# dayne-2stacks/Fingerprint-Matching-Code

Measured on AMD Instinct MI355X. Metric: graph-match pairs/sec @ n=256 kpts, batch=1024, 1 & 8 GPU, higher is better.
Workload: dtype bf16

## Files before the change

fingerprint-matching-code_amd/csrc/gemm.hip:

```cpp
#include "gemm_phase.h"
#include <cstdlib>
#include <cstring>

namespace fpm {
int& gemm_bn256_min();
}
int& gemm_store_sc1_flag();

extern "C" int fpm_gemm(int dtype, const void* A, long lda, long sA, const int* a_rows, const void* B, long ldb,
                        long sB, int M, int N, int K, int batch, int epi, const float* bias, float* Cf, void* Ct,
                        long ldc, long sC, const int* n1, const int* n2, void* stream) {
    using namespace fpm;
    FPM_CHECK_ARG(dtype == 0 || dtype == 1, "gemm: dtype must be 0 (f32) or 1 (bf16)");
    FPM_CHECK_ARG(M >= 0 && N > 0 && K > 0 && batch >= 0, "gemm: bad sizes M=%d N=%d K=%d", M, N, K);
    FPM_CHECK_ARG(K % (dtype ? 8 : 4) == 0, "gemm: K=%d must be a multiple of %d", K, dtype ? 8 : 4);
    FPM_CHECK_ARG(lda % (dtype ? 8 : 4) == 0 && ldb % (dtype ? 8 : 4) == 0, "gemm: lda/ldb must keep rows 16-B aligned");
    FPM_CHECK_ARG((epi != EPI_AFFINITY && epi != EPI_HALF_AFFINITY) || (n1 && n2),
                  "gemm: affinity epilogues need n1/n2");
    FPM_CHECK_ARG(epi >= EPI_STORE && epi <= EPI_HALF_AFFINITY, "gemm: bad epilogue %d", epi);
    if (M == 0 || batch == 0) return 0;
    GemmParams p = {};
    p.A = A; p.lda = lda; p.sA = sA; p.a_rows = a_rows;
    p.B = B; p.ldb = ldb; p.sB = sB; p.sB_seg = 0;
    p.row_scale = nullptr;
// ... 2 lines not shown
    p.epi = epi; p.bias = bias; p.Cf = Cf; p.Ct = Ct; p.ldc = ldc; p.sC = sC; p.n1 = n1; p.n2 = n2;
    hipStream_t st = (hipStream_t)stream;
    const int mt = (M + G2_BM - 1) / G2_BM;
    const bool epi_ok = epi == EPI_STORE || epi == EPI_RELU || (epi == EPI_AFFINITY && Cf && !Ct);
    const bool big = dtype == 1 && M >= G2_BM && K % G2_BK == 0 && N % 8 == 0 && lda % 8 == 0 && ldb % 8 == 0 &&
                     !(Cf && Ct) && (Cf ? ldc % 4 == 0 : ldc % 8 == 0) && epi_ok &&
                     (long)mt * ((N + 127) / 128) * batch >= 128;
    if (big) {
        const int BN = (N % 256 == 0 && (long)mt * (N / 256) * batch >= gemm_bn256_min()) ? 256 : 128;
        p.remap_mtiles = mt;
        dim3 grid(remap_grid_big(N, BN, mt), 1, batch);
        const bool f32 = Cf != nullptr;
        const bool phase = BN == 256 && use_gemm_phase(K);
#define FPM_BIG(BN_, E_, F_)                                                                            \
    do {                                                                                               \
        if (BN_ == 256 && phase) hipLaunchKernelGGL((gemm_phase_kernel<E_, F_>), grid, dim3(G2_THREADS), 0, st, p); \
        else hipLaunchKernelGGL((gemm_big_kernel<BN_, E_, F_>), grid, dim3(G2_THREADS), 0, st, p);      \
    } while (0)
        if (epi == EPI_AFFINITY) {
            if (BN == 256) FPM_BIG(256, EPI_AFFINITY, true); else FPM_BIG(128, EPI_AFFINITY, true);
        } else if (BN == 256) {
            if (epi == EPI_RELU) { if (f32) FPM_BIG(256, EPI_RELU, true); else FPM_BIG(256, EPI_RELU, false); }
            else if (f32) FPM_BIG(256, EPI_STORE, true);
            else {
                const int S = phase ? gemm_walk_strip(p) : 0;
                p.store_sc1 = gemm_store_sc1_flag();
                if (S != 0) gemm_walk_launch(p, S, batch, st);
                else FPM_BIG(256, EPI_STORE, false);
            }
        } else {
            if (epi == EPI_RELU) { if (f32) FPM_BIG(128, EPI_RELU, true); else FPM_BIG(128, EPI_RELU, false); }
// ... 10 lines not shown
}

namespace fpm {
int& gemm_phase_flag() {
    static int on = [] {
        const char* e = getenv("FPM_GEMM_PHASE");
        return e ? atoi(e) : 1;
    }();
    return on;
}

int& gemm_walk_flag() {
    static int v = [] {
        const char* e = getenv("FPM_GEMM_WALK");
        return e ? atoi(e) : GW_AUTO;
    }();
    return v;
}

int gemm_cu_count() {
    static int cus = [] {
        int dev = 0, n = 0;
        if (hipGetDevice(&dev) != hipSuccess ||
            hipDeviceGetAttribute(&n, hipDeviceAttributeMultiprocessorCount, dev) != hipSuccess || n <= 0)
            n = 256;
        return n;
    }();
    return cus;
}

// ... 127 lines not shown
int& gnn_store_sc1_flag();
int& combine_store_sc1_flag();
int& gemm_store_sc1_flag();
int& combine_lds_kb_flag();
int& gnn_mlp_off_flag();
int& outer_sum_vec_flag();
int& gnn_sweeps_flag();
int& scatter_f32_rows_flag();
int& scatter_batch_flag();
int& afau_head_split_flag();

extern "C" int fpm_set_tuning(const char* key, int value) {
    int* f = nullptr;
    if (key && !strcmp(key, "gemm_phase")) f = &fpm::gemm_phase_flag();
    else if (key && !strcmp(key, "gemm_walk")) f = &fpm::gemm_walk_flag();
    else if (key && !strcmp(key, "gemm_bn256_min")) f = &fpm::gemm_bn256_min();
    else if (key && !strcmp(key, "plan_graph")) f = &plan_graph_flag();
    else if (key && !strcmp(key, "combine_npb")) f = &combine_npb_flag();
    else if (key && !strcmp(key, "sinkhorn_bwd_reg")) f = &sinkhorn_bwd_reg_flag();
    else if (key && !strcmp(key, "sinkhorn_fast")) f = &sinkhorn_fast_flag();
    else if (key && !strcmp(key, "sinkhorn_lform")) f = &sinkhorn_lform_flag();
    else if (key && !strcmp(key, "topk_fast")) f = &soft_topk_fast_flag();
    else if (key && !strcmp(key, "afau_attn_v")) f = &afau_attn_v_flag();
    else if (key && !strcmp(key, "gnn_store_sc1")) f = &gnn_store_sc1_flag();
    else if (key && !strcmp(key, "combine_store_sc1")) f = &combine_store_sc1_flag();
    else if (key && !strcmp(key, "gemm_store_sc1")) f = &gemm_store_sc1_flag();
    else if (key && !strcmp(key, "combine_lds_kb")) f = &combine_lds_kb_flag();
    else if (key && !strcmp(key, "gnn_mlp_off")) f = &gnn_mlp_off_flag();
    else if (key && !strcmp(key, "outer_sum_vec")) f = &outer_sum_vec_flag();
    else if (key && !strcmp(key, "gnn_sweeps")) f = &gnn_sweeps_flag();
// ... 175 lines not shown
```

fingerprint-matching-code_amd/csrc/gemm_phase.h:

```cpp
#pragma once
#include <type_traits>
#include "gemm_big.h"

namespace fpm {

constexpr int GP_HALF = 128 * 128;
constexpr int GP_SMEM = g2_max(8 * GP_HALF, G2_BM * (2 * 256 + 16));
constexpr int GP_MIN_KTILES = 2;

#define FPM_VMCNT(N) asm volatile("s_waitcnt vmcnt(" #N ")" ::: "memory")

#ifdef GP_PROBE
__device__ unsigned long long* gp_probe_buf;
#define GP_STAMP(k)                                                                                   \
    do {                                                                                              \
        const unsigned long long t_ = __builtin_amdgcn_s_memtime();                                   \
        if (threadIdx.x == 0 && gp_probe_buf)                                                         \
            gp_probe_buf[((long)blockIdx.z * gridDim.x + blockIdx.x) * 8 + (k)] = t_;                   \
    } while (0)
#else
#define GP_STAMP(k)
#endif

#ifndef GP_STAGGER
#define GP_STAGGER 1
#endif
#ifndef GP_PRIO
#define GP_PRIO 1
#endif
template <int EPI, bool F32OUT, bool DIRECT = false>
__global__ __launch_bounds__(G2_THREADS, 1) void gemm_phase_kernel(GemmParams p) {
    constexpr int BN = 256;
    __shared__ __attribute__((aligned(16))) unsigned char smem[GP_SMEM];
    const int tid = threadIdx.x, lane = tid & 63, wave = tid >> 6;
    const int wr = wave >> 2, wc = wave & 3;
    const int batch = blockIdx.z;

    const int nt = (p.N + BN - 1) / BN;
    const int q = remap_tile(nt, p.remap_mtiles, p.remap_cm > 0 ? p.remap_cm : 4);
    const int mtile = q / nt, ntile = q - mtile * nt;
    if (mtile >= p.remap_mtiles) return;
    int group = 0, row0, row_end;
    if (p.tile_info) {
        group = p.tile_info[2 * mtile];
        if (group < 0) return;
        row0 = p.tile_info[2 * mtile + 1];
        row_end = p.group_off[group + 1];
    } else {
        row0 = mtile * G2_BM;
        row_end = p.M;
// ... 7 lines not shown
    for (int i = 0; i < 2; ++i) {
        const int r = (wave * 2 + i) * 8 + (lane >> 3);
        const int kc = (lane & 7) ^ ((r >> 1) & 7);
#pragma unroll
        for (int h = 0; h < 2; ++h) {
            int gr = row0 + h * 128 + r;
            gr = gr < row_end ? gr : row0;
            const long arow = p.a_rows ? (long)p.a_rows[gr] : (long)gr;
            src[h][i] = A + arow * p.lda + kc * 8;
            const int n = n0 + h * 128 + r < p.N ? n0 + h * 128 + r : p.N - 1;
            src[2 + h][i] = Bg + (long)n * p.ldb + kc * 8;
        }
    }
    auto issue = [&](int j, int slot) {
        const int t = j >> 2;
        unsigned char* dst = smem + ((t & 1) * 4 + slot) * GP_HALF + wave * 2048;
        const int k0 = t * G2_BK;
        __builtin_amdgcn_global_load_lds((gbl_ptr_t)(src[slot][0] + k0), (lds_ptr_t)dst, 16, 0, 0);
        __builtin_amdgcn_global_load_lds((gbl_ptr_t)(src[slot][1] + k0), (lds_ptr_t)(dst + 1024), 16, 0, 0);
    };

    const int xr = (lane >> 1) & 7;
    const int a_off = (wr * 64 + (lane & 15)) * 128;
    const int b_off = (wc * 32 + (lane & 15)) * 128;
    const int s0 = ((lane >> 4) ^ xr) * 16, s1 = ((4 + (lane >> 4)) ^ xr) * 16;

    f32x4_t acc[2][2][4][2];
#pragma unroll
    for (int h = 0; h < 2; ++h)
#pragma unroll
        for (int g = 0; g < 2; ++g)
#pragma unroll
            for (int i = 0; i < 4; ++i)
#pragma unroll
                for (int j = 0; j < 2; ++j) acc[h][g][i][j] = f32x4_t{0.f, 0.f, 0.f, 0.f};
    bf16x8_t a[2][4], b0[2][2], b1[2][2];

    auto read_a = [&](int t, int h) {
        const unsigned char* base = smem + ((t & 1) * 4 + h) * GP_HALF + a_off;
#pragma unroll
        for (int f = 0; f < 4; ++f) {
            a[0][f] = *(const bf16x8_t*)(base + f * 2048 + s0);
            a[1][f] = *(const bf16x8_t*)(base + f * 2048 + s1);
        }
    };
    auto read_b = [&](int t, int g, bf16x8_t (&bb)[2][2]) {
        const unsigned char* base = smem + ((t & 1) * 4 + 2 + g) * GP_HALF + b_off;
#pragma unroll
        for (int f = 0; f < 2; ++f) {
            bb[0][f] = *(const bf16x8_t*)(base + f * 2048 + s0);
            bb[1][f] = *(const bf16x8_t*)(base + f * 2048 + s1);
        }
    };
    auto mfma = [&](f32x4_t (&c)[4][2], bf16x8_t (&bb)[2][2]) {
        __builtin_amdgcn_s_barrier();
        asm volatile("s_waitcnt lgkmcnt(0)" ::: "memory");
        if (GP_PRIO) __builtin_amdgcn_s_setprio(1);
#pragma unroll
        for (int kk = 0; kk < 2; ++kk)
#pragma unroll
            for (int fm = 0; fm < 4; ++fm)
#pragma unroll
                for (int fn = 0; fn < 2; ++fn) {
                    if constexpr (DIRECT)
                        c[fm][fn] = __builtin_amdgcn_mfma_f32_16x16x32_bf16(bb[kk][fn], a[kk][fm], c[fm][fn], 0, 0, 0);
                    else
                        c[fm][fn] = __builtin_amdgcn_mfma_f32_16x16x32_bf16(a[kk][fm], bb[kk][fn], c[fm][fn], 0, 0, 0);
                }
        if (GP_PRIO) __builtin_amdgcn_s_setprio(0);
        __builtin_amdgcn_s_barrier();
    };
    constexpr int SLOT[4] = {0, 2, 3, 1};
    auto ktile = [&](int t, auto VM0, auto VM1, auto VM2, auto VM3, bool iss0, bool iss1, bool iss2, bool iss3) {
        const int phi = 4 * t;
        if constexpr (decltype(VM0)::value == 6) FPM_VMCNT(6);
        else if constexpr (decltype(VM0)::value == 4) FPM_VMCNT(4);
        else if constexpr (decltype(VM0)::value == 2) FPM_VMCNT(2);
        else if constexpr (decltype(VM0)::value == 0) FPM_VMCNT(0);
        if (iss0) issue(phi + 6, SLOT[(0 + 6) & 3]);
        read_a(t, 0);
        read_b(t, 0, b0);
        mfma(acc[0][0], b0);
        if constexpr (decltype(VM1)::value == 6) FPM_VMCNT(6);
        else if constexpr (decltype(VM1)::value == 4) FPM_VMCNT(4);
        else if constexpr (decltype(VM1)::value == 2) FPM_VMCNT(2);
        else if constexpr (decltype(VM1)::value == 0) FPM_VMCNT(0);
        if (iss1) issue(phi + 7, SLOT[(1 + 6) & 3]);
        read_b(t, 1, b1);
        mfma(acc[0][1], b1);
        if constexpr (decltype(VM2)::value == 6) FPM_VMCNT(6);
        else if constexpr (decltype(VM2)::value == 4) FPM_VMCNT(4);
        else if constexpr (decltype(VM2)::value == 2) FPM_VMCNT(2);
        else if constexpr (decltype(VM2)::value == 0) FPM_VMCNT(0);
        if (iss2) issue(phi + 8, SLOT[(2 + 6) & 3]);
        read_a(t, 1);
        mfma(acc[1][1], b1);
        if constexpr (decltype(VM3)::value == 6) FPM_VMCNT(6);
        else if constexpr (decltype(VM3)::value == 4) FPM_VMCNT(4);
        else if constexpr (decltype(VM3)::value == 2) FPM_VMCNT(2);
        else if constexpr (decltype(VM3)::value == 0) FPM_VMCNT(0);
        if (iss3) issue(phi + 9, SLOT[(3 + 6) & 3]);
        mfma(acc[1][0], b0);
    };
    using V6 = std::integral_constant<int, 6>;
    using V4 = std::integral_constant<int, 4>;
    using V2 = std::integral_constant<int, 2>;
    using V0 = std::integral_constant<int, 0>;
    using VN = std::integral_constant<int, -1>;

    GP_STAMP(0);
    const int ktiles = p.K / G2_BK;
#pragma unroll
    for (int j = 0; j < 6; ++j) issue(j, SLOT[j & 3]);
    FPM_VMCNT(8);
    __builtin_amdgcn_s_barrier();
    GP_STAMP(1);
    if (GP_STAGGER && wr == 1) __builtin_amdgcn_s_barrier();

    int t = 0;
    for (; t < ktiles - 2; ++t) ktile(t, V6{}, V6{}, V6{}, V6{}, true, true, true, true);
    ktile(t, V6{}, V6{}, V6{}, V4{}, true, true, false, false);
    ktile(t + 1, V2{}, V0{}, VN{}, VN{}, false, false, false, false);
    if (GP_STAGGER && wr == 0) __builtin_amdgcn_s_barrier();
    __syncthreads();
    GP_STAMP(2);

    int n1b = 0, n2b = 0;
    if (EPI == EPI_AFFINITY) { n1b = p.n1[batch]; n2b = p.n2[batch]; }
    if constexpr (DIRECT) {
        static_assert(!F32OUT && EPI == EPI_STORE, "DIRECT: bf16 output, plain store");
        bf16_t* Ct = (bf16_t*)p.Ct + (long)batch * p.sC;
        const int cl = wc * 32 + 4 * (lane >> 4);
#pragma unroll
        for (int h = 0; h < 2; ++h)
#pragma unroll
            for (int fm = 0; fm < 4; ++fm) {
                const int r = row0 + h * 128 + wr * 64 + fm * 16 + (lane & 15);
// ... 125 lines not shown

constexpr int GW_SMEM = 8 * GP_HALF;
constexpr int GW_MAX_S = 2;

__host__ __device__ inline int gemm_walk_rule(int tiles, int wgs, int cus) {
    const long r1 = ((long)tiles * wgs + cus - 1) / cus, r2 = ((long)((tiles + 1) / 2) * wgs + cus - 1) / cus;
    return 2 * r2 * 7 <= r1 * 8 ? 2 : 1;
}

#ifdef GP_PROBE
#define GW_STAMP(k) do { if (ti == 0) GP_STAMP(k); } while (0)
#else
#define GW_STAMP(k)
#endif

template <bool SC1>
__global__ __launch_bounds__(G2_THREADS, 1) void gemm_walk_kernel(GemmParams p) {
    constexpr int BN = 256;
    __shared__ __attribute__((aligned(16))) unsigned char smem[GW_SMEM];
    const int tid = threadIdx.x, lane = tid & 63, wave = tid >> 6;
    const int wr = wave >> 2, wc = wave & 3;
    const int batch = blockIdx.z;

    const int nt = p.N / BN;
    int mtiles = p.remap_mtiles;
    if (p.tile_count) mtiles = *p.tile_count < mtiles ? *p.tile_count : mtiles;
    const int S = p.walk > 0 ? p.walk : gemm_walk_rule(mtiles, nt * (int)gridDim.z, p.walk_cus);
    const int strips = (mtiles + S - 1) / S;
    const int i = blockIdx.x >> 3;
    const int strip = (i / nt) * 8 + (blockIdx.x & 7), ntile = i % nt;
    if (strip >= strips) return;
    int t_row0[GW_MAX_S], t_rend[GW_MAX_S], t_grp[GW_MAX_S];
    unsigned ok = 0;
#pragma unroll
    for (int j = 0; j < GW_MAX_S; ++j) {
        const int mt = strip * S + j;
// ... 23 lines not shown
    auto pick = [&](const int (&t)[GW_MAX_S], int j) __attribute__((always_inline)) {
        return j == 0 ? t[0] : t[1];
    };
    int m = next_valid(0);

    const int n0 = ntile * BN;
    const bf16_t* A = (const bf16_t*)p.A + (long)batch * p.sA;
    const unsigned char* Bb = (const unsigned char*)((const bf16_t*)p.B + (long)batch * p.sB);
    bf16_t* Ct = (bf16_t*)p.Ct + (long)batch * p.sC;

    auto tile_at = [&](int j, int& row0, int& row_end, const unsigned char*& bg) __attribute__((always_inline)) {
        row0 = pick(t_row0, j);
        row_end = pick(t_rend, j);
        bg = Bb + (long)pick(t_grp, j) * p.sB_seg * 2;
    };
    auto a_rows_of = [&](int row0, int row_end, int (&ar)[2][2]) __attribute__((always_inline)) {
#pragma unroll
        for (int i = 0; i < 2; ++i)
#pragma unroll
            for (int h = 0; h < 2; ++h) {
                int gr = row0 + h * 128 + (wave * 2 + i) * 8 + (lane >> 3);
                gr = gr < row_end ? gr : row0;
                ar[h][i] = p.a_rows ? p.a_rows[gr] : gr;
            }
    };
    const uint32_t kc16 = (uint32_t)(((lane & 7) ^ (lane >> 4)) * 16);
    uint32_t b_off[2];
#pragma unroll
    for (int i = 0; i < 2; ++i)
        b_off[i] = (uint32_t)((n0 + (wave * 2 + i) * 8 + (lane >> 3)) * (uint32_t)p.ldb * 2) + (kc16 ^ (i * 64));
    const uint32_t lda2 = (uint32_t)p.lda * 2, bhalf = 128 * (uint32_t)p.ldb * 2;
    const unsigned char* Ab = (const unsigned char*)A;

    int row0, row_end, row0n = 0, row_endn = 0;
    const unsigned char *bg, *bgn = nullptr;
    int ar[2][2], arn[2][2];

    auto issue = [&](int slot, int buf, const int (&rows)[2][2], const unsigned char* bgrp, int k0) __attribute__((always_inline)) {
        unsigned char* dst = smem + (buf * 4 + slot) * GP_HALF + wave * 2048;
        if (slot < 2) {
            const unsigned char* ab = Ab + 2 * k0;
#pragma unroll
            for (int i = 0; i < 2; ++i)
                __builtin_amdgcn_global_load_lds(
                    (gbl_ptr_t)(ab + ((uint64_t)(uint32_t)rows[slot][i] * lda2 + (kc16 ^ (i * 64)))),
                    (lds_ptr_t)(dst + i * 1024), 16, 0, 0);
        } else {
            const unsigned char* b = bgrp + 2 * k0 + (slot - 2) * bhalf;
            __builtin_amdgcn_global_load_lds((gbl_ptr_t)(b + b_off[0]), (lds_ptr_t)dst, 16, 0, 0);
            __builtin_amdgcn_global_load_lds((gbl_ptr_t)(b + b_off[1]), (lds_ptr_t)(dst + 1024), 16, 0, 0);
        }
    };

    const int xr = (lane >> 1) & 7;
    const int a_off = (wr * 64 + (lane & 15)) * 128;
    const int b_offl = (wc * 32 + (lane & 15)) * 128;
    const int s0 = ((lane >> 4) ^ xr) * 16, s1 = ((4 + (lane >> 4)) ^ xr) * 16;

    f32x4_t acc[2][2][4][2];
    auto zero_acc = [&]() __attribute__((always_inline)) {
#pragma unroll
        for (int h = 0; h < 2; ++h)
#pragma unroll
            for (int g = 0; g < 2; ++g)
#pragma unroll
                for (int i = 0; i < 4; ++i)
#pragma unroll
                    for (int j = 0; j < 2; ++j) acc[h][g][i][j] = f32x4_t{0.f, 0.f, 0.f, 0.f};
    };
    bf16x8_t a[2][4], b0[2][2], b1[2][2];

    auto read_a = [&](int u, int h) __attribute__((always_inline)) {
        const unsigned char* base = smem + ((u & 1) * 4 + h) * GP_HALF + a_off;
#pragma unroll
        for (int f = 0; f < 4; ++f) {
            a[0][f] = *(const bf16x8_t*)(base + f * 2048 + s0);
            a[1][f] = *(const bf16x8_t*)(base + f * 2048 + s1);
        }
    };
    auto read_b = [&](int u, int g, bf16x8_t (&bb)[2][2]) __attribute__((always_inline)) {
        const unsigned char* base = smem + ((u & 1) * 4 + 2 + g) * GP_HALF + b_offl;
#pragma unroll
        for (int f = 0; f < 2; ++f) {
            bb[0][f] = *(const bf16x8_t*)(base + f * 2048 + s0);
            bb[1][f] = *(const bf16x8_t*)(base + f * 2048 + s1);
        }
    };
    auto mfma = [&](f32x4_t (&c)[4][2], bf16x8_t (&bb)[2][2]) __attribute__((always_inline)) {
        __builtin_amdgcn_s_barrier();
        asm volatile("s_waitcnt lgkmcnt(0)" ::: "memory");
        if (GP_PRIO) __builtin_amdgcn_s_setprio(1);
#pragma unroll
        for (int kk = 0; kk < 2; ++kk)
#pragma unroll
            for (int fm = 0; fm < 4; ++fm)
#pragma unroll
                for (int fn = 0; fn < 2; ++fn)
                    c[fm][fn] = __builtin_amdgcn_mfma_f32_16x16x32_bf16(bb[kk][fn], a[kk][fm], c[fm][fn], 0, 0, 0);
        if (GP_PRIO) __builtin_amdgcn_s_setprio(0);
        __builtin_amdgcn_s_barrier();
    };
    constexpr int NONE = 0, CUR = 1, NEXT = 2;
    auto wait = [&](int v) __attribute__((always_inline)) {
        if (v == 6) FPM_VMCNT(6);
        else if (v == 4) FPM_VMCNT(4);
        else if (v == 2) FPM_VMCNT(2);
        else if (v == 0) FPM_VMCNT(0);
    };
    auto iss = [&](int mode, int slot, int buf, int k0) __attribute__((always_inline)) {
        if (mode == CUR) issue(slot, buf, ar, bg, k0);
        else if (mode == NEXT) issue(slot, buf, arn, bgn, 0);
    };
    auto ktile = [&](int u, int k1, int VM0, int VM1, int VM2, int VM3, int M01, int M23) __attribute__((always_inline)) {
        asm volatile("" : "+s"(k1));
        wait(VM0);
        iss(M01, 3, (u + 1) & 1, k1);
        read_a(u, 0);
        read_b(u, 0, b0);
        mfma(acc[0][0], b0);
        wait(VM1);
        iss(M01, 1, (u + 1) & 1, k1);
        read_b(u, 1, b1);
        mfma(acc[0][1], b1);
        wait(VM2);
        iss(M23, 0, u & 1, k1 + G2_BK);
        read_a(u, 1);
        mfma(acc[1][1], b1);
        wait(VM3);
        iss(M23, 2, u & 1, k1 + G2_BK);
        mfma(acc[1][0], b0);
    };

    auto epilogue = [&](int buf, auto hb) __attribute__((always_inline)) {
        constexpr bool HB = decltype(hb)::value;
        unsigned char* img = smem + buf * (4 * GP_HALF);
        int tid_ = tid;
        asm volatile("" : "+v"(tid_));
        const int lane = tid_ & 63, wr = tid_ >> 8, wc = (tid_ >> 6) & 3;
        int wbase[2];
#pragma unroll
        for (int fn = 0; fn < 2; ++fn)
            wbase[fn] = (wr * 64 + (lane & 15)) * 512 + (((wc * 4 + fn * 2 + (lane >> 5)) ^ (lane & 7)) << 4) +
                        ((lane >> 4) & 1) * 8;
        const int rb_r = tid_ >> 5, rb_c = tid_ & 31;
        const int rbase = rb_r * 512 + ((rb_c ^ (rb_r & 7)) << 4);
// ... 32 lines not shown
                    }
                }
            } else {
#pragma unroll
                for (int it = 0; it < 8; ++it) {
                    const uint4 v = *(const uint4*)(img + rbase + it * 8192);
                    if (rbeg + it * 16 < row_end) *(uint4*)(Ct + (long)(rbeg + it * 16) * p.ldc + n0 + rb_c * 8) = v;
                }
            }
            asm volatile("s_waitcnt lgkmcnt(0)" ::: "memory");
            __builtin_amdgcn_s_barrier();
        }
    };

    const int T = p.K / G2_BK;
    tile_at(m, row0, row_end, bg);
    a_rows_of(row0, row_end, ar);
    int mn = next_valid(m + 1);
    if (mn < m_end) {
        tile_at(mn, row0n, row_endn, bgn);
        a_rows_of(row0n, row_endn, arn);
    }
    issue(0, 0, ar, bg, 0);
    issue(2, 0, ar, bg, 0);
    issue(3, 0, ar, bg, 0);
    issue(1, 0, ar, bg, 0);
    issue(0, 1, ar, bg, G2_BK);
    issue(2, 1, ar, bg, G2_BK);
    zero_acc();
    FPM_VMCNT(8);
    __builtin_amdgcn_s_barrier();

    int u = 0;
#ifdef GP_PROBE
    int ti = 0;
#endif
    for (;;) {
        const bool has_next = mn < m_end;
        GW_STAMP(0);
        if (GP_STAGGER && wr == 1) __builtin_amdgcn_s_barrier();
        int k1 = G2_BK;
        for (int t = 0; t < T - 2; ++t, ++u, k1 += G2_BK) ktile(u, k1, 6, 6, 6, 6, CUR, CUR);
        ktile(u, k1, 6, 6, 6, has_next ? 6 : 4, CUR, has_next ? NEXT : NONE);
        GW_STAMP(1);
        ktile(u + 1, 0, has_next ? 6 : 2, has_next ? 6 : 0, -1, -1, has_next ? NEXT : NONE, NONE);
        ++u;
        if (GP_STAGGER && wr == 0) __builtin_amdgcn_s_barrier();
        GW_STAMP(2);
        if (p.bias) epilogue(u & 1, std::true_type{});
        else epilogue(u & 1, std::false_type{});
        GW_STAMP(3);
        if (!has_next) break;
        m = mn; mn = m_end;
        row0 = row0n; row_end = row_endn; bg = bgn;
#pragma unroll
        for (int h = 0; h < 2; ++h)
#pragma unroll
            for (int i = 0; i < 2; ++i) ar[h][i] = arn[h][i];
        issue(0, u & 1, ar, bg, G2_BK);
        issue(2, u & 1, ar, bg, G2_BK);
        FPM_VMCNT(4);
        zero_acc();
        __builtin_amdgcn_s_barrier();
        GW_STAMP(4);
        ++u;
#ifdef GP_PROBE
        ++ti;
#endif
    }
}

#undef FPM_VMCNT

int& gemm_phase_flag();
inline bool use_gemm_phase(int K) { return gemm_phase_flag() != 0 && K / G2_BK >= GP_MIN_KTILES; }

constexpr int GW_AUTO = 8;
int& gemm_walk_flag();
int gemm_cu_count();
inline int gemm_walk_strip(const GemmParams& p) {
    const int f = gemm_walk_flag();
    if (f <= 1 || !use_gemm_phase(p.K) || p.N % 256 != 0 || !p.Ct || p.Cf || p.epi != EPI_STORE) return 0;
    if ((long)p.N * p.ldb * 2 >= (1L << 31) || (long)G2_BM * p.ldc * 2 >= (1L << 31) || p.lda >= (1L << 31)) return 0;
    return f < GW_AUTO ? 2 : GW_AUTO;
}
inline void gemm_walk_launch(GemmParams p, int S, int batch, hipStream_t st) {
    const long nt = p.N / 256;
    p.walk_cus = gemm_cu_count();
    p.walk = S == 2 || p.remap_mtiles * nt * batch >= 8L * gemm_cu_count() ? 2 : 0;
    const int strips = p.walk ? (p.remap_mtiles + 1) / 2 : p.remap_mtiles;
    const dim3 grid((unsigned)((strips + 7) / 8 * 8 * nt), 1, batch);
    if (p.store_sc1) hipLaunchKernelGGL((gemm_walk_kernel<true>), grid, dim3(G2_THREADS), 0, st, p);
    else hipLaunchKernelGGL((gemm_walk_kernel<false>), grid, dim3(G2_THREADS), 0, st, p);
}

}
```

fingerprint-matching-code_amd/csrc/spline.hip:

```cpp
#include "gemm_phase.h"

#include <vector>

namespace {

struct ProfRec {
    hipEvent_t a, b;
    int slot;
};
bool g_prof_on = false;
std::vector<ProfRec> g_prof;
int* g_prof_rows = nullptr;
constexpr int PROF_MAX = 4096;

constexpr int NCELL = 26;

struct PlanLayout {
    long mask, indeg, dslot, basis_e, grp_e, blk_cnt, cell_off, rowid, arows, tile_info, tile_info2, dst_ptr, csr_e,
        nbr_local, rows4, basis4, total;
    long nblk, max_rows, max_tiles, max_tiles2;
};

__host__ __device__ inline long al(long x) { return (x + 255) & ~255L; }

// ... 1134 lines not shown
        if (dtype == 1) p.tile_info = (const int*)(w + L.tile_info2);
        const int walk = dtype == 1 ? gemm_walk_strip(p) : 0;
        p.tile_count = (const int*)(w + L.cell_off) + NCELL + 2;
        dim3 grid(dtype == 0 ? remap_grid(D, p.remap_mtiles) : remap_grid256(D, p.remap_mtiles), 1, 1);
        ProfRec rec = {nullptr, nullptr, (int)g_prof.size()};
        if (g_prof_on && !g_prof_rows) (void)hipMalloc(&g_prof_rows, PROF_MAX * sizeof(int));
        if (g_prof_on && g_prof_rows && rec.slot < PROF_MAX) {
            (void)hipMemcpyAsync(g_prof_rows + rec.slot, w + L.cell_off + NCELL * sizeof(int), sizeof(int),
                                 hipMemcpyDeviceToDevice, st);
            (void)hipEventCreate(&rec.a);
            (void)hipEventCreate(&rec.b);
            (void)hipEventRecord(rec.a, st);
        }
        if (dtype == 0) hipLaunchKernelGGL((gemm_kernel<float, false>), grid, dim3(GTHREADS), 0, st, p);
        else if (walk != 0) gemm_walk_launch(p, walk, 1, st);
        else if (use_gemm_phase(D)) hipLaunchKernelGGL((gemm_phase_kernel<EPI_STORE, false>), grid, dim3(G2_THREADS), 0, st, p);
        else hipLaunchKernelGGL((gemm_big_kernel<256, EPI_STORE, false>), grid, dim3(G2_THREADS), 0, st, p);
        if (g_prof_on && g_prof_rows && rec.slot < PROF_MAX) {
            (void)hipEventRecord(rec.b, st);
            g_prof.push_back(rec);
        }
    }
    {
        const long graphs = (num_nodes + nmax - 1) / nmax;
        const int npb = combine_npb_flag();
#define FPM_COMB(T_, N_)                                                                                         \
    do {                                                                                                         \
        const dim3 cg((unsigned)(((graphs + 7) / 8) * 8 * ((nmax + N_ - 1) / N_)));                              \
        const size_t lds = (size_t)combine_lds_kb_flag() * 1024;                                                 \
        if (combine_store_sc1_flag() && !(mode >> 1))                                                            \
            hipLaunchKernelGGL((combine_kernel<T_, N_, false, 16>), cg, dim3(64 * N_), lds, st, (const T_*)y_ws, \
// ... 328 lines not shown
    }
    GemmParams p = {};
    p.A = dtype == 0 ? (const void*)dY : (const void*)dY_op; p.lda = D; p.a_rows = nullptr;
    p.B = Wb; p.ldb = D; p.sB_seg = (long)D * D;
    p.M = (int)L.max_rows; p.N = D; p.K = D; p.nseg = 1;
    p.group_off = (const int*)(w + L.cell_off);
    p.epi = EPI_STORE; p.ldc = D; p.Cf = dXrows;
    if (dtype == 0) {
        p.tile_info = (const int*)(w + L.tile_info);
        p.remap_mtiles = (int)L.max_tiles;
        hipLaunchKernelGGL((gemm_kernel<float, false>), dim3(remap_grid(D, p.remap_mtiles)), dim3(GTHREADS), 0, st, p);
    } else {
        p.tile_info = (const int*)(w + L.tile_info2);
        p.remap_mtiles = (int)L.max_tiles2;
        dim3 grid(remap_grid256(D, p.remap_mtiles));
        if (use_gemm_phase(D)) hipLaunchKernelGGL((gemm_phase_kernel<EPI_STORE, true>), grid, dim3(G2_THREADS), 0, st, p);
        else hipLaunchKernelGGL((gemm_big_kernel<256, EPI_STORE, true>), grid, dim3(G2_THREADS), 0, st, p);
    }
    hipLaunchKernelGGL(node_rows_sum_kernel, dim3(nb), dim3(256), 0, st, dXrows, (const int*)(w + L.rowid), num_nodes,
                       accumulate, dX);
    return check_launch("fpm_spline_conv_bwd_data");
}

namespace {

template <typename TO, bool TRANS>
__global__ __launch_bounds__(256) void spline_w_pack_kernel(const float* __restrict__ weight,
                                                            const float* __restrict__ root, int K, int Cin, int Cout,
                                                            TO* __restrict__ out) {
    __shared__ float t[64][65];
    const int k = blockIdx.z;
// ... 40 lines not shown
```

Measured before the change: 32570.

## Balance LDS reads across GEMM phase quarters by prefetching next B tile

Reorders the global-to-LDS stream slots and moves the first B-fragment read of each k-tile into the previous k-tile's last quarter. This spreads LDS reads more evenly across the four MFMA phases. B register buffers alternate between k-tiles through a swap flag, and an odd/even prologue handles the tile count parity. The phase and walk kernels now share a common k-tile helper. A probe-only per-phase clock is added, and the balanced variant is on by default through a new FPM_GEMM_BALANCE flag. The risk is extra register pressure and subtle pipeline hazards from the reordered slot timing.

```diff
diff --git a/fingerprint-matching-code_amd/csrc/gemm.hip b/fingerprint-matching-code_amd/csrc/gemm.hip
--- a/fingerprint-matching-code_amd/csrc/gemm.hip
+++ b/fingerprint-matching-code_amd/csrc/gemm.hip
@@ -40,7 +40,7 @@
         const bool phase = BN == 256 && use_gemm_phase(K);
 #define FPM_BIG(BN_, E_, F_)                                                                            \
     do {                                                                                               \
-        if (BN_ == 256 && phase) hipLaunchKernelGGL((gemm_phase_kernel<E_, F_>), grid, dim3(G2_THREADS), 0, st, p); \
+        if (BN_ == 256 && phase) gemm_phase_launch<E_, F_>(p, grid, st);                                \
         else hipLaunchKernelGGL((gemm_big_kernel<BN_, E_, F_>), grid, dim3(G2_THREADS), 0, st, p);      \
     } while (0)
         if (epi == EPI_AFFINITY) {
@@ -81,6 +81,14 @@
     static int v = [] {
         const char* e = getenv("FPM_GEMM_WALK");
         return e ? atoi(e) : GW_AUTO;
+    }();
+    return v;
+}
+
+int& gemm_balance_flag() {
+    static int v = [] {
+        const char* e = getenv("FPM_GEMM_BALANCE");
+        return e ? atoi(e) : 1;
     }();
     return v;
 }
@@ -238,6 +246,7 @@
     int* f = nullptr;
     if (key && !strcmp(key, "gemm_phase")) f = &fpm::gemm_phase_flag();
     else if (key && !strcmp(key, "gemm_walk")) f = &fpm::gemm_walk_flag();
+    else if (key && !strcmp(key, "gemm_balance")) f = &fpm::gemm_balance_flag();
     else if (key && !strcmp(key, "gemm_bn256_min")) f = &fpm::gemm_bn256_min();
     else if (key && !strcmp(key, "plan_graph")) f = &plan_graph_flag();
     else if (key && !strcmp(key, "combine_npb")) f = &combine_npb_flag();
diff --git a/fingerprint-matching-code_amd/csrc/gemm_phase.h b/fingerprint-matching-code_amd/csrc/gemm_phase.h
--- a/fingerprint-matching-code_amd/csrc/gemm_phase.h
+++ b/fingerprint-matching-code_amd/csrc/gemm_phase.h
@@ -18,8 +18,51 @@
         if (threadIdx.x == 0 && gp_probe_buf)                                                         \
             gp_probe_buf[((long)blockIdx.z * gridDim.x + blockIdx.x) * 8 + (k)] = t_;                   \
     } while (0)
+__device__ unsigned* gp_phase_buf;
+struct GpClock {
+    unsigned last, sum[4][3], n;
+    static __device__ __forceinline__ unsigned now() {
+        unsigned long long t;
+        __builtin_amdgcn_sched_barrier(0);
+        asm volatile("s_memtime %0\n\ts_waitcnt lgkmcnt(0)" : "=s"(t)::"memory");
+        __builtin_amdgcn_sched_barrier(0);
+        return (unsigned)t;
+    }
+    __device__ __forceinline__ void start() {
+        n = 0;
+#pragma unroll
+        for (int q = 0; q < 4; ++q)
+#pragma unroll
+            for (int k = 0; k < 3; ++k) sum[q][k] = 0;
+        last = now();
+    }
+    __device__ __forceinline__ void resume() { last = now(); }
+    __device__ __forceinline__ void mark(int q, int part) {
+        const unsigned t = now();
+        sum[q][part] += t - last;
+        last = t;
+    }
+    __device__ __forceinline__ void ktile_done() { ++n; }
+    __device__ __forceinline__ void store() const {
+        if ((threadIdx.x & 255) == 0 && gp_phase_buf) {
+            unsigned* o = gp_phase_buf + (((long)blockIdx.z * gridDim.x + blockIdx.x) * 2 + (threadIdx.x >> 8)) * 16;
+#pragma unroll
+            for (int q = 0; q < 4; ++q)
+#pragma unroll
+                for (int k = 0; k < 3; ++k) o[q * 3 + k] = sum[q][k];
+            o[12] = n;
+        }
+    }
+};
 #else
 #define GP_STAMP(k)
+struct GpClock {
+    __device__ __forceinline__ void start() {}
+    __device__ __forceinline__ void resume() {}
+    __device__ __forceinline__ void mark(int, int) {}
+    __device__ __forceinline__ void ktile_done() {}
+    __device__ __forceinline__ void store() const {}
+};
 #endif
 
 #ifndef GP_STAGGER
@@ -28,12 +71,100 @@
 #ifndef GP_PRIO
 #define GP_PRIO 1
 #endif
-template <int EPI, bool F32OUT, bool DIRECT = false>
+
+__device__ __forceinline__ void gp_wait(int v) {
+    if (v == 6) FPM_VMCNT(6);
+    else if (v == 4) FPM_VMCNT(4);
+    else if (v == 2) FPM_VMCNT(2);
+    else if (v == 0) FPM_VMCNT(0);
+}
+
+template <bool SWAP>
+struct GpTile {
+    const unsigned char* smem;
+    int a_off, b_off, s0, s1;
+    __device__ __forceinline__ GpTile(const unsigned char* sm, int lane, int wr, int wc) : smem(sm) {
+        const int xr = (lane >> 1) & 7;
+        a_off = (wr * 64 + (lane & 15)) * 128;
+        b_off = (wc * 32 + (lane & 15)) * 128;
+        s0 = ((lane >> 4) ^ xr) * 16;
+        s1 = ((4 + (lane >> 4)) ^ xr) * 16;
+    }
+    __device__ __forceinline__ void read_a(int u, int h, bf16x8_t (&a)[2][4]) const {
+        const unsigned char* base = smem + ((u & 1) * 4 + h) * GP_HALF + a_off;
+#pragma unroll
+        for (int f = 0; f < 4; ++f) {
+            a[0][f] = *(const bf16x8_t*)(base + f * 2048 + s0);
+            a[1][f] = *(const bf16x8_t*)(base + f * 2048 + s1);
+        }
+    }
+    __device__ __forceinline__ void read_b(int u, int g, bf16x8_t (&bb)[2][2]) const {
+        const unsigned char* base = smem + ((u & 1) * 4 + 2 + g) * GP_HALF + b_off;
+#pragma unroll
+        for (int f = 0; f < 2; ++f) {
+            bb[0][f] = *(const bf16x8_t*)(base + f * 2048 + s0);
+            bb[1][f] = *(const bf16x8_t*)(base + f * 2048 + s1);
+        }
+    }
+    __device__ __forceinline__ void mfma(GpClock& clk, int q, f32x4_t (&c)[4][2], const bf16x8_t (&a)[2][4],
+                                         const bf16x8_t (&bb)[2][2]) const {
+        __builtin_amdgcn_s_barrier();
+        asm volatile("s_waitcnt lgkmcnt(0)" ::: "memory");
+        clk.mark(q, 1);
+        if (GP_PRIO) __builtin_amdgcn_s_setprio(1);
+#pragma unroll
+        for (int kk = 0; kk < 2; ++kk)
+#pragma unroll
+            for (int fm = 0; fm < 4; ++fm)
+#pragma unroll
+                for (int fn = 0; fn < 2; ++fn) {
+                    if constexpr (SWAP)
+                        c[fm][fn] = __builtin_amdgcn_mfma_f32_16x16x32_bf16(bb[kk][fn], a[kk][fm], c[fm][fn], 0, 0, 0);
+                    else
+                        c[fm][fn] = __builtin_amdgcn_mfma_f32_16x16x32_bf16(a[kk][fm], bb[kk][fn], c[fm][fn], 0, 0, 0);
+                }
+        if (GP_PRIO) __builtin_amdgcn_s_setprio(0);
+        __builtin_amdgcn_s_barrier();
+        clk.mark(q, 2);
+    }
+};
+
+template <bool BAL>
+__device__ __forceinline__ constexpr int gp_stream_slot(int pos) {
+    return pos == 0 ? (BAL ? 2 : 0) : pos == 1 ? (BAL ? 0 : 2) : pos == 2 ? 3 : 1;
+}
+
+template <bool BAL, bool SWAP, class Stage>
+__device__ __forceinline__ void gp_ktile(const GpTile<SWAP>& T, GpClock& clk, int u, bool pre, Stage&& stage,
+                                         f32x4_t (&acc)[2][2][4][2], bf16x8_t (&a)[2][4], bf16x8_t (&bx)[2][2],
+                                         bf16x8_t (&by)[2][2]) {
+    stage(std::integral_constant<int, 0>{});
+    clk.mark(0, 0);
+    T.read_a(u, 0, a);
+    if constexpr (!BAL) T.read_b(u, 0, bx);
+    T.mfma(clk, 0, acc[0][0], a, bx);
+    stage(std::integral_constant<int, 1>{});
+    clk.mark(1, 0);
+    T.read_b(u, 1, by);
+    T.mfma(clk, 1, acc[0][1], a, by);
+    stage(std::integral_constant<int, 2>{});
+    clk.mark(2, 0);
+    T.read_a(u, 1, a);
+    T.mfma(clk, 2, acc[1][1], a, by);
+    stage(std::integral_constant<int, 3>{});
+    clk.mark(3, 0);
+    if (BAL && pre) T.read_b(u + 1, 0, by);
+    T.mfma(clk, 3, acc[1][0], a, bx);
+    clk.ktile_done();
+}
+
+template <int EPI, bool F32OUT, bool DIRECT = false, bool BAL = true>
 __global__ __launch_bounds__(G2_THREADS, 1) void gemm_phase_kernel(GemmParams p) {
     constexpr int BN = 256;
     __shared__ __attribute__((aligned(16))) unsigned char smem[GP_SMEM];
     const int tid = threadIdx.x, lane = tid & 63, wave = tid >> 6;
     const int wr = wave >> 2, wc = wave & 3;
+    const int wave_s = __builtin_amdgcn_readfirstlane(wave);
     const int batch = blockIdx.z;
 
     const int nt = (p.N + BN - 1) / BN;
@@ -71,17 +202,14 @@
     }
     auto issue = [&](int j, int slot) {
         const int t = j >> 2;
-        unsigned char* dst = smem + ((t & 1) * 4 + slot) * GP_HALF + wave * 2048;
+        unsigned char* dst = smem + ((t & 1) * 4 + slot) * GP_HALF + wave_s * 2048;
         const int k0 = t * G2_BK;
         __builtin_amdgcn_global_load_lds((gbl_ptr_t)(src[slot][0] + k0), (lds_ptr_t)dst, 16, 0, 0);
         __builtin_amdgcn_global_load_lds((gbl_ptr_t)(src[slot][1] + k0), (lds_ptr_t)(dst + 1024), 16, 0, 0);
     };
 
-    const int xr = (lane >> 1) & 7;
-    const int a_off = (wr * 64 + (lane & 15)) * 128;
-    const int b_off = (wc * 32 + (lane & 15)) * 128;
-    const int s0 = ((lane >> 4) ^ xr) * 16, s1 = ((4 + (lane >> 4)) ^ xr) * 16;
-
+    const GpTile<DIRECT> T(smem, lane, wr, wc);
+    GpClock clk;
     f32x4_t acc[2][2][4][2];
 #pragma unroll
     for (int h = 0; h < 2; ++h)
@@ -93,91 +221,44 @@
                 for (int j = 0; j < 2; ++j) acc[h][g][i][j] = f32x4_t{0.f, 0.f, 0.f, 0.f};
     bf16x8_t a[2][4], b0[2][2], b1[2][2];
 
-    auto read_a = [&](int t, int h) {
-        const unsigned char* base = smem + ((t & 1) * 4 + h) * GP_HALF + a_off;
-#pragma unroll
-        for (int f = 0; f < 4; ++f) {
-            a[0][f] = *(const bf16x8_t*)(base + f * 2048 + s0);
-            a[1][f] = *(const bf16x8_t*)(base + f * 2048 + s1);
-        }
-    };
-    auto read_b = [&](int t, int g, bf16x8_t (&bb)[2][2]) {
-        const unsigned char* base = smem + ((t & 1) * 4 + 2 + g) * GP_HALF + b_off;
-#pragma unroll
-        for (int f = 0; f < 2; ++f) {
-            bb[0][f] = *(const bf16x8_t*)(base + f * 2048 + s0);
-            bb[1][f] = *(const bf16x8_t*)(base + f * 2048 + s1);
-        }
-    };
-    auto mfma = [&](f32x4_t (&c)[4][2], bf16x8_t (&bb)[2][2]) {
-        __builtin_amdgcn_s_barrier();
-        asm volatile("s_waitcnt lgkmcnt(0)" ::: "memory");
-        if (GP_PRIO) __builtin_amdgcn_s_setprio(1);
-#pragma unroll
-        for (int kk = 0; kk < 2; ++kk)
-#pragma unroll
-            for (int fm = 0; fm < 4; ++fm)
-#pragma unroll
-                for (int fn = 0; fn < 2; ++fn) {
-                    if constexpr (DIRECT)
-                        c[fm][fn] = __builtin_amdgcn_mfma_f32_16x16x32_bf16(bb[kk][fn], a[kk][fm], c[fm][fn], 0, 0, 0);
-                    else
-                        c[fm][fn] = __builtin_amdgcn_mfma_f32_16x16x32_bf16(a[kk][fm], bb[kk][fn], c[fm][fn], 0, 0, 0);
-                }
-        if (GP_PRIO) __builtin_amdgcn_s_setprio(0);
-        __builtin_amdgcn_s_barrier();
-    };
-    constexpr int SLOT[4] = {0, 2, 3, 1};
-    auto ktile = [&](int t, auto VM0, auto VM1, auto VM2, auto VM3, bool iss0, bool iss1, bool iss2, bool iss3) {
-        const int phi = 4 * t;
-        if constexpr (decltype(VM0)::value == 6) FPM_VMCNT(6);
-        else if constexpr (decltype(VM0)::value == 4) FPM_VMCNT(4);
-        else if constexpr (decltype(VM0)::value == 2) FPM_VMCNT(2);
-        else if constexpr (decltype(VM0)::value == 0) FPM_VMCNT(0);
-        if (iss0) issue(phi + 6, SLOT[(0 + 6) & 3]);
-        read_a(t, 0);
-        read_b(t, 0, b0);
-        mfma(acc[0][0], b0);
-        if constexpr (decltype(VM1)::value == 6) FPM_VMCNT(6);
-        else if constexpr (decltype(VM1)::value == 4) FPM_VMCNT(4);
-        else if constexpr (decltype(VM1)::value == 2) FPM_VMCNT(2);
-        else if constexpr (decltype(VM1)::value == 0) FPM_VMCNT(0);
-        if (iss1) issue(phi + 7, SLOT[(1 + 6) & 3]);
-        read_b(t, 1, b1);
-        mfma(acc[0][1], b1);
-        if constexpr (decltype(VM2)::value == 6) FPM_VMCNT(6);
-        else if constexpr (decltype(VM2)::value == 4) FPM_VMCNT(4);
-        else if constexpr (decltype(VM2)::value == 2) FPM_VMCNT(2);
-        else if constexpr (decltype(VM2)::value == 0) FPM_VMCNT(0);
-        if (iss2) issue(phi + 8, SLOT[(2 + 6) & 3]);
-        read_a(t, 1);
-        mfma(acc[1][1], b1);
-        if constexpr (decltype(VM3)::value == 6) FPM_VMCNT(6);
-        else if constexpr (decltype(VM3)::value == 4) FPM_VMCNT(4);
-        else if constexpr (decltype(VM3)::value == 2) FPM_VMCNT(2);
-        else if constexpr (decltype(VM3)::value == 0) FPM_VMCNT(0);
-        if (iss3) issue(phi + 9, SLOT[(3 + 6) & 3]);
-        mfma(acc[1][0], b0);
-    };
-    using V6 = std::integral_constant<int, 6>;
-    using V4 = std::integral_constant<int, 4>;
-    using V2 = std::integral_constant<int, 2>;
-    using V0 = std::integral_constant<int, 0>;
-    using VN = std::integral_constant<int, -1>;
+    auto ktile = [&](int t, int v0, int v1, int v2, int v3, int ni, bool pre, bool swap) {
+        auto stage = [&](auto qc) {
+            constexpr int Q = decltype(qc)::value;
+            gp_wait(Q == 0 ? v0 : Q == 1 ? v1 : Q == 2 ? v2 : v3);
+            if (Q < ni) issue(4 * t + Q + 6, gp_stream_slot<BAL>((Q + 2) & 3));
+        };
+        if (BAL && swap) gp_ktile<BAL>(T, clk, t, pre, stage, acc, a, b1, b0);
+        else gp_ktile<BAL>(T, clk, t, pre, stage, acc, a, b0, b1);
+    };
 
     GP_STAMP(0);
     const int ktiles = p.K / G2_BK;
-#pragma unroll
-    for (int j = 0; j < 6; ++j) issue(j, SLOT[j & 3]);
+    const bool odd = BAL && ((ktiles - 2) & 1);
+#pragma unroll
+    for (int j = 0; j < 6; ++j) issue(j, gp_stream_slot<BAL>(j & 3));
     FPM_VMCNT(8);
     __builtin_amdgcn_s_barrier();
     GP_STAMP(1);
+    if constexpr (BAL) {
+        if (odd) T.read_b(0, 0, b1);
+        else T.read_b(0, 0, b0);
+    }
     if (GP_STAGGER && wr == 1) __builtin_amdgcn_s_barrier();
+    clk.start();
 
     int t = 0;
-    for (; t < ktiles - 2; ++t) ktile(t, V6{}, V6{}, V6{}, V6{}, true, true, true, true);
-    ktile(t, V6{}, V6{}, V6{}, V4{}, true, true, false, false);
-    ktile(t + 1, V2{}, V0{}, VN{}, VN{}, false, false, false, false);
+    if constexpr (BAL) {
+        if (odd) { ktile(0, 6, 6, 6, 6, 4, true, true); t = 1; }
+        for (; t < ktiles - 2; t += 2) {
+            ktile(t, 6, 6, 6, 6, 4, true, false);
+            ktile(t + 1, 6, 6, 6, 6, 4, true, true);
+        }
+    } else {
+        for (; t < ktiles - 2; ++t) ktile(t, 6, 6, 6, 6, 4, false, false);
+    }
+    ktile(t, 6, 6, 6, 4, 2, true, false);
+    ktile(t + 1, 2, 0, -1, -1, 0, false, true);
+    clk.store();
     if (GP_STAGGER && wr == 0) __builtin_amdgcn_s_barrier();
     __syncthreads();
     GP_STAMP(2);
@@ -333,12 +414,13 @@
 #define GW_STAMP(k)
 #endif
 
-template <bool SC1>
+template <bool SC1, bool BAL = true>
 __global__ __launch_bounds__(G2_THREADS, 1) void gemm_walk_kernel(GemmParams p) {
     constexpr int BN = 256;
     __shared__ __attribute__((aligned(16))) unsigned char smem[GW_SMEM];
     const int tid = threadIdx.x, lane = tid & 63, wave = tid >> 6;
     const int wr = wave >> 2, wc = wave & 3;
+    const int wave_s = __builtin_amdgcn_readfirstlane(wave);
     const int batch = blockIdx.z;
 
     const int nt = p.N / BN;
@@ -392,49 +474,49 @@
         row_end = pick(t_rend, j);
         bg = Bb + (long)pick(t_grp, j) * p.sB_seg * 2;
     };
-    auto a_rows_of = [&](int row0, int row_end, int (&ar)[2][2]) __attribute__((always_inline)) {
+    const uint32_t kc16 = (uint32_t)(((lane & 7) ^ (lane >> 4)) * 16);
+    const uint32_t lda2 = (uint32_t)p.lda * 2, bhalf = 128 * (uint32_t)p.ldb * 2;
+    auto a_rows_of = [&](int row0, int row_end, uint32_t (&ar)[2][2]) __attribute__((always_inline)) {
 #pragma unroll
         for (int i = 0; i < 2; ++i)
 #pragma unroll
             for (int h = 0; h < 2; ++h) {
                 int gr = row0 + h * 128 + (wave * 2 + i) * 8 + (lane >> 3);
                 gr = gr < row_end ? gr : row0;
-                ar[h][i] = p.a_rows ? p.a_rows[gr] : gr;
-            }
-    };
-    const uint32_t kc16 = (uint32_t)(((lane & 7) ^ (lane >> 4)) * 16);
+                ar[h][i] = (uint32_t)(p.a_rows ? p.a_rows[gr] : gr);
+            }
+    };
     uint32_t b_off[2];
 #pragma unroll
     for (int i = 0; i < 2; ++i)
         b_off[i] = (uint32_t)((n0 + (wave * 2 + i) * 8 + (lane >> 3)) * (uint32_t)p.ldb * 2) + (kc16 ^ (i * 64));
-    const uint32_t lda2 = (uint32_t)p.lda * 2, bhalf = 128 * (uint32_t)p.ldb * 2;
     const unsigned char* Ab = (const unsigned char*)A;
 
     int row0, row_end, row0n = 0, row_endn = 0;
     const unsigned char *bg, *bgn = nullptr;
-    int ar[2][2], arn[2][2];
-
-    auto issue = [&](int slot, int buf, const int (&rows)[2][2], const unsigned char* bgrp, int k0) __attribute__((always_inline)) {
-        unsigned char* dst = smem + (buf * 4 + slot) * GP_HALF + wave * 2048;
+    uint32_t ar[2][2], arn[2][2];
+
+    auto issue = [&](int slot, int buf, uint32_t (&rows)[2][2], const unsigned char* bgrp, int k0) __attribute__((always_inline)) {
+        unsigned char* dst = smem + (buf * 4 + slot) * GP_HALF + wave_s * 2048;
         if (slot < 2) {
             const unsigned char* ab = Ab + 2 * k0;
 #pragma unroll
             for (int i = 0; i < 2; ++i)
                 __builtin_amdgcn_global_load_lds(
-                    (gbl_ptr_t)(ab + ((uint64_t)(uint32_t)rows[slot][i] * lda2 + (kc16 ^ (i * 64)))),
+                    (gbl_ptr_t)(ab + ((uint64_t)rows[slot][i] * lda2 + (kc16 ^ (i * 64)))),
                     (lds_ptr_t)(dst + i * 1024), 16, 0, 0);
         } else {
             const unsigned char* b = bgrp + 2 * k0 + (slot - 2) * bhalf;
-            __builtin_amdgcn_global_load_lds((gbl_ptr_t)(b + b_off[0]), (lds_ptr_t)dst, 16, 0, 0);
-            __builtin_amdgcn_global_load_lds((gbl_ptr_t)(b + b_off[1]), (lds_ptr_t)(dst + 1024), 16, 0, 0);
-        }
-    };
-
-    const int xr = (lane >> 1) & 7;
-    const int a_off = (wr * 64 + (lane & 15)) * 128;
-    const int b_offl = (wc * 32 + (lane & 15)) * 128;
-    const int s0 = ((lane >> 4) ^ xr) * 16, s1 = ((4 + (lane >> 4)) ^ xr) * 16;
-
+#pragma unroll
+            for (int i = 0; i < 2; ++i) {
+                asm volatile("" : "+v"(b_off[i]));
+                __builtin_amdgcn_global_load_lds((gbl_ptr_t)(b + b_off[i]), (lds_ptr_t)(dst + i * 1024), 16, 0, 0);
+            }
+        }
+    };
+
+    const GpTile<true> F(smem, lane, wr, wc);
+    GpClock clk;
     f32x4_t acc[2][2][4][2];
     auto zero_acc = [&]() __attribute__((always_inline)) {
 #pragma unroll
@@ -448,65 +530,23 @@
     };
     bf16x8_t a[2][4], b0[2][2], b1[2][2];
 
-    auto read_a = [&](int u, int h) __attribute__((always_inline)) {
-        const unsigned char* base = smem + ((u & 1) * 4 + h) * GP_HALF + a_off;
-#pragma unroll
-        for (int f = 0; f < 4; ++f) {
-            a[0][f] = *(const bf16x8_t*)(base + f * 2048 + s0);
-            a[1][f] = *(const bf16x8_t*)(base + f * 2048 + s1);
-        }
-    };
-    auto read_b = [&](int u, int g, bf16x8_t (&bb)[2][2]) __attribute__((always_inline)) {
-        const unsigned char* base = smem + ((u & 1) * 4 + 2 + g) * GP_HALF + b_offl;
-#pragma unroll
-        for (int f = 0; f < 2; ++f) {
-            bb[0][f] = *(const bf16x8_t*)(base + f * 2048 + s0);
-            bb[1][f] = *(const bf16x8_t*)(base + f * 2048 + s1);
-        }
-    };
-    auto mfma = [&](f32x4_t (&c)[4][2], bf16x8_t (&bb)[2][2]) __attribute__((always_inline)) {
-        __builtin_amdgcn_s_barrier();
-        asm volatile("s_waitcnt lgkmcnt(0)" ::: "memory");
-        if (GP_PRIO) __builtin_amdgcn_s_setprio(1);
-#pragma unroll
-        for (int kk = 0; kk < 2; ++kk)
-#pragma unroll
-            for (int fm = 0; fm < 4; ++fm)
-#pragma unroll
-                for (int fn = 0; fn < 2; ++fn)
-                    c[fm][fn] = __builtin_amdgcn_mfma_f32_16x16x32_bf16(bb[kk][fn], a[kk][fm], c[fm][fn], 0, 0, 0);
-        if (GP_PRIO) __builtin_amdgcn_s_setprio(0);
-        __builtin_amdgcn_s_barrier();
-    };
     constexpr int NONE = 0, CUR = 1, NEXT = 2;
-    auto wait = [&](int v) __attribute__((always_inline)) {
-        if (v == 6) FPM_VMCNT(6);
-        else if (v == 4) FPM_VMCNT(4);
-        else if (v == 2) FPM_VMCNT(2);
-        else if (v == 0) FPM_VMCNT(0);
-    };
     auto iss = [&](int mode, int slot, int buf, int k0) __attribute__((always_inline)) {
         if (mode == CUR) issue(slot, buf, ar, bg, k0);
         else if (mode == NEXT) issue(slot, buf, arn, bgn, 0);
     };
-    auto ktile = [&](int u, int k1, int VM0, int VM1, int VM2, int VM3, int M01, int M23) __attribute__((always_inline)) {
+    auto ktile = [&](int u, int k1, int VM0, int VM1, int VM2, int VM3, int M01, int M23, bool pre, bool swap) __attribute__((always_inline)) {
         asm volatile("" : "+s"(k1));
-        wait(VM0);
-        iss(M01, 3, (u + 1) & 1, k1);
-        read_a(u, 0);
-        read_b(u, 0, b0);
-        mfma(acc[0][0], b0);
-        wait(VM1);
-        iss(M01, 1, (u + 1) & 1, k1);
-        read_b(u, 1, b1);
-        mfma(acc[0][1], b1);
-        wait(VM2);
-        iss(M23, 0, u & 1, k1 + G2_BK);
-        read_a(u, 1);
-        mfma(acc[1][1], b1);
-        wait(VM3);
-        iss(M23, 2, u & 1, k1 + G2_BK);
-        mfma(acc[1][0], b0);
+        const int k2 = k1 + G2_BK;
+        auto stage = [&](auto qc) __attribute__((always_inline)) {
+            constexpr int Q = decltype(qc)::value;
+            constexpr int slot = gp_stream_slot<BAL>((Q + 2) & 3);
+            gp_wait(Q == 0 ? VM0 : Q == 1 ? VM1 : Q == 2 ? VM2 : VM3);
+            if (Q < 2) iss(M01, slot, (u + 1) & 1, k1);
+            else iss(M23, slot, u & 1, k2);
+        };
+        if (BAL && swap) gp_ktile<BAL>(F, clk, u, pre, stage, acc, a, b1, b0);
+        else gp_ktile<BAL>(F, clk, u, pre, stage, acc, a, b0, b1);
     };
 
     auto epilogue = [&](int buf, auto hb) __attribute__((always_inline)) {
@@ -569,6 +609,7 @@
     };
 
     const int T = p.K / G2_BK;
+    const bool odd = BAL && ((T - 2) & 1);
     tile_at(m, row0, row_end, bg);
     a_rows_of(row0, row_end, ar);
     int mn = next_valid(m + 1);
@@ -576,12 +617,8 @@
         tile_at(mn, row0n, row_endn, bgn);
         a_rows_of(row0n, row_endn, arn);
     }
-    issue(0, 0, ar, bg, 0);
-    issue(2, 0, ar, bg, 0);
-    issue(3, 0, ar, bg, 0);
-    issue(1, 0, ar, bg, 0);
-    issue(0, 1, ar, bg, G2_BK);
-    issue(2, 1, ar, bg, G2_BK);
+#pragma unroll
+    for (int j = 0; j < 6; ++j) issue(gp_stream_slot<BAL>(j & 3), j >> 2, ar, bg, (j >> 2) * G2_BK);
     zero_acc();
     FPM_VMCNT(8);
     __builtin_amdgcn_s_barrier();
@@ -590,15 +627,29 @@
 #ifdef GP_PROBE
     int ti = 0;
 #endif
+    clk.start();
     for (;;) {
         const bool has_next = mn < m_end;
         GW_STAMP(0);
+        if constexpr (BAL) {
+            if (odd) F.read_b(u, 0, b1);
+            else F.read_b(u, 0, b0);
+        }
         if (GP_STAGGER && wr == 1) __builtin_amdgcn_s_barrier();
-        int k1 = G2_BK;
-        for (int t = 0; t < T - 2; ++t, ++u, k1 += G2_BK) ktile(u, k1, 6, 6, 6, 6, CUR, CUR);
-        ktile(u, k1, 6, 6, 6, has_next ? 6 : 4, CUR, has_next ? NEXT : NONE);
+        clk.resume();
+        int k1 = G2_BK, t = 0;
+        if constexpr (BAL) {
+            if (odd) { ktile(u, k1, 6, 6, 6, 6, CUR, CUR, true, true); t = 1; ++u; k1 += G2_BK; }
+            for (; t < T - 2; t += 2, u += 2, k1 += 2 * G2_BK) {
+                ktile(u, k1, 6, 6, 6, 6, CUR, CUR, true, false);
+                ktile(u + 1, k1 + G2_BK, 6, 6, 6, 6, CUR, CUR, true, true);
+            }
+        } else {
+            for (; t < T - 2; ++t, ++u, k1 += G2_BK) ktile(u, k1, 6, 6, 6, 6, CUR, CUR, false, false);
+        }
+        ktile(u, k1, 6, 6, 6, has_next ? 6 : 4, CUR, has_next ? NEXT : NONE, true, false);
         GW_STAMP(1);
-        ktile(u + 1, 0, has_next ? 6 : 2, has_next ? 6 : 0, -1, -1, has_next ? NEXT : NONE, NONE);
+        ktile(u + 1, 0, has_next ? 6 : 2, has_next ? 6 : 0, -1, -1, has_next ? NEXT : NONE, NONE, false, true);
         ++u;
         if (GP_STAGGER && wr == 0) __builtin_amdgcn_s_barrier();
         GW_STAMP(2);
@@ -612,8 +663,8 @@
         for (int h = 0; h < 2; ++h)
 #pragma unroll
             for (int i = 0; i < 2; ++i) ar[h][i] = arn[h][i];
-        issue(0, u & 1, ar, bg, G2_BK);
-        issue(2, u & 1, ar, bg, G2_BK);
+        issue(gp_stream_slot<BAL>(0), u & 1, ar, bg, G2_BK);
+        issue(gp_stream_slot<BAL>(1), u & 1, ar, bg, G2_BK);
         FPM_VMCNT(4);
         zero_acc();
         __builtin_amdgcn_s_barrier();
@@ -623,12 +674,20 @@
         ++ti;
 #endif
     }
+    clk.store();
 }
 
 #undef FPM_VMCNT
 
 int& gemm_phase_flag();
 inline bool use_gemm_phase(int K) { return gemm_phase_flag() != 0 && K / G2_BK >= GP_MIN_KTILES; }
+
+int& gemm_balance_flag();
+template <int EPI, bool F32OUT>
+inline void gemm_phase_launch(const GemmParams& p, dim3 grid, hipStream_t st) {
+    if (gemm_balance_flag()) hipLaunchKernelGGL((gemm_phase_kernel<EPI, F32OUT, false, true>), grid, dim3(G2_THREADS), 0, st, p);
+    else hipLaunchKernelGGL((gemm_phase_kernel<EPI, F32OUT, false, false>), grid, dim3(G2_THREADS), 0, st, p);
+}
 
 constexpr int GW_AUTO = 8;
 int& gemm_walk_flag();
@@ -645,8 +704,9 @@
     p.walk = S == 2 || p.remap_mtiles * nt * batch >= 8L * gemm_cu_count() ? 2 : 0;
     const int strips = p.walk ? (p.remap_mtiles + 1) / 2 : p.remap_mtiles;
     const dim3 grid((unsigned)((strips + 7) / 8 * 8 * nt), 1, batch);
-    if (p.store_sc1) hipLaunchKernelGGL((gemm_walk_kernel<true>), grid, dim3(G2_THREADS), 0, st, p);
-    else hipLaunchKernelGGL((gemm_walk_kernel<false>), grid, dim3(G2_THREADS), 0, st, p);
-}
-
-}
+    void (*const kern[4])(GemmParams) = {gemm_walk_kernel<false, false>, gemm_walk_kernel<false, true>,
+                                         gemm_walk_kernel<true, false>, gemm_walk_kernel<true, true>};
+    hipLaunchKernelGGL(kern[(p.store_sc1 ? 2 : 0) | (gemm_balance_flag() ? 1 : 0)], grid, dim3(G2_THREADS), 0, st, p);
+}
+
+}
diff --git a/fingerprint-matching-code_amd/csrc/spline.hip b/fingerprint-matching-code_amd/csrc/spline.hip
--- a/fingerprint-matching-code_amd/csrc/spline.hip
+++ b/fingerprint-matching-code_amd/csrc/spline.hip
@@ -1172,7 +1172,7 @@
         }
         if (dtype == 0) hipLaunchKernelGGL((gemm_kernel<float, false>), grid, dim3(GTHREADS), 0, st, p);
         else if (walk != 0) gemm_walk_launch(p, walk, 1, st);
-        else if (use_gemm_phase(D)) hipLaunchKernelGGL((gemm_phase_kernel<EPI_STORE, false>), grid, dim3(G2_THREADS), 0, st, p);
+        else if (use_gemm_phase(D)) gemm_phase_launch<EPI_STORE, false>(p, grid, st);
         else hipLaunchKernelGGL((gemm_big_kernel<256, EPI_STORE, false>), grid, dim3(G2_THREADS), 0, st, p);
         if (g_prof_on && g_prof_rows && rec.slot < PROF_MAX) {
             (void)hipEventRecord(rec.b, st);
@@ -1531,7 +1531,7 @@
         p.tile_info = (const int*)(w + L.tile_info2);
         p.remap_mtiles = (int)L.max_tiles2;
         dim3 grid(remap_grid256(D, p.remap_mtiles));
-        if (use_gemm_phase(D)) hipLaunchKernelGGL((gemm_phase_kernel<EPI_STORE, true>), grid, dim3(G2_THREADS), 0, st, p);
+        if (use_gemm_phase(D)) gemm_phase_launch<EPI_STORE, true>(p, grid, st);
         else hipLaunchKernelGGL((gemm_big_kernel<256, EPI_STORE, true>), grid, dim3(G2_THREADS), 0, st, p);
     }
     hipLaunchKernelGGL(node_rows_sum_kernel, dim3(nb), dim3(256), 0, st, dXrows, (const int*)(w + L.rowid), num_nodes,
```

Result: no change. 33020, median of 6 (+1.4%).
